# VIS4ROB-lab/HyperSLAM

Hardware: AMD Instinct MI355X
Metric: residual blocks linearised per second (LM iteration = linearise + Schur + solve + update), 128-control-point window (higher is better)
Workload: dtype f64

## Files before the change

hyperslam_amd/csrc/host_structure.hpp:

```cpp
#pragma once
#include <algorithm>
#include <cmath>
#include <cstdint>
#include <numeric>
#include <string>
#include <vector>

#include "../../include/hyperslam_hip.h"
#include "device_math.hpp"

namespace hs {

inline double h_binom(int n, int r) {
  if (r < 0 || r > n) return 0.0;
  double v = 1.0;
  for (int i = 1; i <= r; ++i) v = v * (n - r + i) / i;
  return v;
}

inline hsd::BasisCoef make_basis_coef(int k) {
  hsd::BasisCoef b;
  for (double& v : b.c) v = 0.0;
  std::vector<double> M(size_t(k) * k, 0.0);
  double fact = 1.0;
// ... 189 lines not shown

inline void order_chunks_for_dispatch(const VisualStructure& vs, int k, int n_cu, std::vector<int>* ch_desc, int n) {
  if (n <= 1 || n_cu <= 0) return;
  std::vector<int> weight(n), order(n);
  std::vector<int> cnt;
  for (int c = 0; c < n; ++c) {
    const int* d = ch_desc->data() + 8 * c;
    cnt.assign(size_t(vs.bw) + k + 1, 0);
    for (int q = d[3]; q < d[3] + d[4]; ++q) {
      const int o = vs.first[q] - d[2];
      if (o >= 0 && o < vs.bw) cnt[o]++;
    }
    int run = 0, best = 0;
    for (int o = 0; o < vs.bw + k; ++o) {
      run += (o < vs.bw ? cnt[o] : 0) - (o >= k ? cnt[o - k] : 0);
      best = std::max(best, run);
    }
    weight[c] = best, order[c] = c;
  }
  std::stable_sort(order.begin(), order.end(), [&](int a, int b) { return weight[a] > weight[b]; });
  std::vector<int> slot_chunk(n, -1);
  if (n > n_cu && n <= 2 * n_cu) {
    const int n_lone = 2 * n_cu - n, n_pair = n - n_cu;
    for (int i = 0; i < n_lone; ++i) slot_chunk[n_pair + i] = order[i];
    for (int i = 0; i < n_pair; ++i) slot_chunk[i] = order[n_lone + i], slot_chunk[n_cu + i] = order[n - 1 - i];
  } else {
    for (int i = 0; i < n; ++i) slot_chunk[i] = order[i];
  }
  std::vector<int> out(ch_desc->size(), 0);
  for (int w = 0; w < n; ++w) std::copy(ch_desc->begin() + 8 * slot_chunk[w], ch_desc->begin() + 8 * slot_chunk[w] + 8, out.begin() + 8 * w);
  ch_desc->swap(out);
}

template <class LdsBytes>
inline bool choose_build_geometry(int k, int R0, int L0, size_t lds_two, size_t lds_one, LdsBytes lds_bytes, int* R, int* L) {
  for (const size_t cap : {lds_two, lds_one}) {
    int r = R0, l = L0;
    while (lds_bytes(r, l) > cap && l > 4) --l;
    while (lds_bytes(r, l) > cap && r > 64) r -= 32;
    if (lds_bytes(r, l) <= cap) {
      *R = r, *L = l;
      return true;
    }
  }
  (void)k;
  return false;
}

}
```

hyperslam_amd/csrc/host_tables.hpp:

```cpp
#pragma once
#include <dlfcn.h>
#include <hip/hip_runtime.h>
#include <rccl/rccl.h>

#include <array>
#include <cstdio>
#include <cstdlib>
#include <chrono>
#include <cstring>
#include <string>
#include <mutex>
#include <vector>

#include "host_structure.hpp"
#include "kernels.hpp"

using namespace hs;

namespace {

struct UploadBatch {
  struct Seg {
    unsigned long long dst, off, bytes;
  };
// ... 224 lines not shown
  const void* zeroed_ptr[5] = {nullptr, nullptr, nullptr, nullptr, nullptr};

  VisualStructure vs;
  std::vector<int> pr_order;
  std::vector<int> pr_first, pr_seg_ptr;

  DBuf<double> d_cp, d_cp_cand, d_cam, d_sensor, d_lm, d_lm_cand;
  DBuf<uint8_t> d_cp_const, d_lm_const;
  DBuf<int> d_lm_ptr, d_lm_cfirst, d_lm_ncp, d_lm_yoff, d_cf_ptr;
  DBuf<double> d_lm_scale, d_lm_L, d_lm_yhat, d_lm_sb, d_lm_D2, d_lm_part, d_lm_gmax, d_gabs, d_Y;
  DBuf<double> d_v_stamp, d_v_meas, d_v_rec, d_v_rec_alt;
  DBuf<int> d_v_lm, d_v_info, d_v_first, d_v_pos, d_v_seg_ptr, d_v_dbgpos;
  DBuf<double> d_p_stamp, d_p_meas, d_p_rec;
  DBuf<double> d_i_stamp, d_i_meas, d_i_rec, d_bias_g, d_bias_a, d_bias_g_cand, d_bias_a_cand, d_gravity, d_gravity_cand;
  DBuf<int> d_i_first, d_i_first_bias, d_i_seg_ptr;
  DBuf<ImuParams> d_imu;
  std::vector<int> in_order, in_first, in_first_bias, in_seg_ptr, in_bias_ptr;
  int nb_ine = 0;
  DBuf<int> d_p_sensor, d_p_first, d_p_seg_ptr;
  DBuf<double> d_scale_p, d_Sb, d_Ub, d_Ubk, d_g_s, d_g_full, d_D2p, d_step_p, d_delta_p;
  DBuf<double> d_cost_part, d_cand_part, d_norm_part, d_dbg, d_dbg_cost;
  DBuf<DevState> d_state;
  DBuf<double> d_xbuf, d_xpart, d_segP, d_grpQ, d_Qw, d_Yt, d_gravity_part;
  int yt_stride = 0;
  bool wide_q = false;
  DBuf<double> d_Vb, d_Vb2, d_yt, d_yt2;
  DBuf<double> d_Mb, d_Mb2;
  DBuf<double> d_Sb2, d_g2, d_Ub2, d_Ubk2, d_ybuf2, d_win, d_xsol;
  DBuf<unsigned> d_join;
  DBuf<double> d_dense_ut;
  DBuf<double> d_bf_handover;
  unsigned join_epoch = 0;
  DBuf<int> d_gw_ptr, d_gw_cf, d_sw_ptr, d_sw_seg;
  int n_seg_wg = 0, n_group_wg = 0;
  bool fused = false;
  int dense_border_nb = -1;
  bool bookkeep = false;
  int build_R = 0, build_L = 0;
  size_t build_lds = 0;
  DBuf<int> d_ch_ptr, d_ch_desc;
  DBuf<double> d_ch_gmax;
  std::vector<int> h_ch_ptr, h_gw_ptr, h_gw_cf, h_ch_desc;
  DBuf<double> d_ybuf, d_scale_b, d_Spb, d_Sbb, d_gb_s, d_D2b, d_Zb, d_Cb, d_hb, d_xb, d_delta_b, d_bias_g_snap, d_bias_a_snap, d_gravity_snap;
  DBuf<int> d_i_bias_ptr, d_bfwd_start;
  int n_split = 1;
  int rank = 0, world = 1, min_bw = 0;
  DBuf<double> d_cp_snap, d_lm_snap;
  bool has_snapshot = false;
  DevState* h_state = nullptr;
  bool cov_valid = false;
  int cov_np = 0, cov_ncb = 0, cov_nb = 0, cov_nlm = 0;
  DBuf<double> d_cov_U, d_cov_sig, d_cov_Z, d_cov_X, d_cov_C, d_cov_Li, d_cov_band, d_cov_pb, d_cov_bb, d_cov_lm;
  DBuf<uint8_t> d_cov_const;
  DBuf<int> d_cov_status, d_cov_lm_status;
  int nc = 0;
  std::vector<int> calib_map;
  DBuf<int> d_calib_map;
  DBuf<double> d_calib_rec, d_calib_Yc, d_calib_part, d_cam_cand;
  DBuf<int> d_calib_bfwd;
  int ni = 0;
  std::vector<int> imucal_map;
  DBuf<int> d_imucal_map;
  DBuf<double> d_imucal_rec, d_imucal_part;
  bool imu_estimation = false;
  bool imu_covariance = false;
  bool imu_estimated() const { return ni > 0 && imu_estimation; }
// ... 530 lines not shown
    const int n_seg_ = p->n_cp - k + 1, nca = 6 * k, ntile = vs.bw * (vs.bw + 1) / 2;
    std::vector<int> sw_ptr(n_seg_ + 1, 0), sw_seg;
    for (int f = 0; f < n_seg_; ++f) {
      const int load = (p->fused ? 0 : vs.seg_ptr[f + 1] - vs.seg_ptr[f]) + 3 * (p->pr_seg_ptr[f + 1] - p->pr_seg_ptr[f]) +
                       (p->in_seg_ptr.empty() ? 0 : 3 * (p->in_seg_ptr[f + 1] - p->in_seg_ptr[f]));
      const int nw = p->fused ? (load + 95) / 96 : std::max(1, (load + 95) / 96);
      sw_ptr[f + 1] = sw_ptr[f] + nw;
      for (int w = 0; w < nw; ++w) sw_seg.push_back(f);
    }
    p->n_seg_wg = sw_ptr[n_seg_];
    sw_seg.push_back(0);
    HIP_TRY(p->d_sw_ptr.upload(sw_ptr, s));
    HIP_TRY(p->d_sw_seg.upload(sw_seg, s));
    const int per_wg = 12;
    std::vector<int> gw_ptr(p->n_cp + 1, 0), gw_cf;
    if (!(what & hs_problem::kVis)) {
    } else if (p->fused) {
      HIP_TRY(p->d_gw_ptr.upload(p->h_gw_ptr, s));
      HIP_TRY(p->d_gw_cf.upload(p->h_gw_cf, s));
      HIP_TRY(p->d_ch_ptr.upload(p->h_ch_ptr, s));
      HIP_TRY(p->d_ch_desc.upload(p->h_ch_desc, s));
      p->n_group_wg = int(p->h_ch_ptr.size()) - 1;
    } else {
      for (int c = 0; c < p->n_cp; ++c) {
        const int cnt = vs.cf_ptr[c + 1] - vs.cf_ptr[c], nw = (cnt + per_wg - 1) / per_wg;
        gw_ptr[c + 1] = gw_ptr[c] + nw;
        for (int w = 0; w < nw; ++w) gw_cf.push_back(c);
      }
      p->n_group_wg = gw_ptr[p->n_cp];
      gw_cf.push_back(0);
      HIP_TRY(p->d_gw_ptr.upload(gw_ptr, s));
      HIP_TRY(p->d_gw_cf.upload(gw_cf, s));
    }
    HIP_TRY(p->d_segP.reserve(size_t(p->n_seg_wg) * (size_t(nca) * nca + nca) + 1));
    HIP_TRY(p->d_grpQ.reserve(size_t(p->n_group_wg) * (size_t(ntile) * 36 + (p->fused ? 3 : 1) * 6 * vs.bw) + 1));
    {
      const char* env = std::getenv("HS_WIDE_Q");
      p->wide_q = p->fused && ntile > kBlock && !(env && std::atoi(env) == 0);
      if (p->wide_q) {
        HIP_TRY(p->d_Qw.reserve(size_t(6) * p->n_cp * (6 * vs.bw + 1) + 1));
        p->yt_stride = (p->n_lm + 63) / 64 * 64;
        HIP_TRY(p->d_Yt.reserve(size_t(18) * p->n_cp * p->yt_stride + 2));
      }
    }
  }
  HIP_TRY(p->d_state.reserve(1));

  Tables& T = p->T;
  std::memset(&T, 0, sizeof(T));
  p->dense_border_nb = -1;
  T.sp = Spline{k, p->n_cp, p->t0, p->dt, 1.0 / p->dt, p->rot_const, p->trans_const};
  T.basis = make_basis_coef(k);
  T.cp = p->d_cp.p, T.cp_cand = p->d_cp_cand.p, T.cp_const = p->d_cp_const.p;
  T.cam = p->d_cam.p, T.n_cam = p->n_cam, T.sensor = p->d_sensor.p;
  T.n_lm = p->n_lm, T.lm = p->d_lm.p, T.lm_cand = p->d_lm_cand.p, T.lm_const = p->d_lm_const.p;
  T.lm_ptr = p->d_lm_ptr.p, T.lm_cfirst = p->d_lm_cfirst.p, T.lm_ncp = p->d_lm_ncp.p, T.lm_yoff = p->d_lm_yoff.p, T.cf_ptr = p->d_cf_ptr.p;
  T.lm_scale = p->d_lm_scale.p, T.lm_L = p->d_lm_L.p, T.lm_yhat = p->d_lm_yhat.p, T.lm_sb = p->d_lm_sb.p, T.lm_D2 = p->d_lm_D2.p;
  T.lm_part = p->d_lm_part.p, T.n_lm_part = p->fused ? p->nb_vis : (p->n_lm + kBlock / 64 - 1) / (kBlock / 64), T.lm_gmax = p->d_lm_gmax.p, T.Y = p->d_Y.p;
  {
    int n_obs = p->n_lm;
    while (n_obs > 0 && vs.lm_ptr[n_obs] == vs.lm_ptr[n_obs - 1]) --n_obs;
    T.n_obs_lm = n_obs;
  }
  T.n_vis = n_vis, T.v_stamp = p->d_v_stamp.p, T.v_meas = p->d_v_meas.p, T.v_lm = p->d_v_lm.p, T.v_info = p->d_v_info.p;
  T.v_first = p->d_v_first.p, T.v_pos = p->d_v_pos.p, T.v_rec = p->d_v_rec.p, T.v_rec_alt = p->d_v_rec_alt.p, T.v_seg_ptr = p->d_v_seg_ptr.p;
  T.n_pri = n_pri, T.p_stamp = p->d_p_stamp.p, T.p_meas = p->d_p_meas.p, T.p_sensor = p->d_p_sensor.p, T.p_first = p->d_p_first.p;
  T.p_rec = p->d_p_rec.p, T.p_seg_ptr = p->d_p_seg_ptr.p;
  T.n_ine = n_ine, T.i_stamp = p->d_i_stamp.p, T.i_meas = p->d_i_meas.p, T.i_first = p->d_i_first.p, T.i_first_bias = p->d_i_first_bias.p;
  T.i_rec = p->d_i_rec.p, T.i_seg_ptr = p->d_i_seg_ptr.p, T.imu = p->d_imu.p;
  T.bias_basis = make_basis_coef(p->kb), T.kb = p->kb, T.n_bias = p->has_imu ? p->n_bias : 0, T.bias_t0 = p->bias_t0, T.bias_dt = p->bias_dt;
  T.bias_g = p->d_bias_g.p, T.bias_a = p->d_bias_a.p, T.bias_g_cand = p->d_bias_g_cand.p, T.bias_a_cand = p->d_bias_a_cand.p;
  T.gravity = p->d_gravity.p, T.gravity_cand = p->d_gravity_cand.p, T.bias_const = p->bias_const, T.gravity_const = p->gravity_const;
  T.inertial_literal = p->inertial_mode == HS_INERTIAL_AS_REFERENCE;
  T.nb = (p->has_imu ? 6 * p->n_bias + 2 : 0) + p->ni + p->nc;
  T.nc = p->nc, T.calib_map = p->d_calib_map.p, T.calib_rec = p->d_calib_rec.p, T.calib_Yc = p->d_calib_Yc.p, T.calib_part = p->d_calib_part.p;
  T.n_seg = n_seg, T.bw = vs.bw, T.np = np;
  T.scale_p = p->d_scale_p.p, T.Sb = p->d_Sb.p, T.Ub = p->d_Ub.p, T.Ubk = p->d_Ubk.p, T.g_s = p->d_g_s.p, T.g_full = p->d_g_full.p, T.D2p = p->d_D2p.p, T.gabs = p->d_gabs.p;
  T.step_p = p->d_step_p.p, T.delta_p = p->d_delta_p.p;
  T.cost_part = p->d_cost_part.p, T.cand_part = p->d_cand_part.p, T.n_cost_part = p->nb_vis + p->nb_pri + p->nb_ine;
  if (size_t(T.n_cost_part) > p->d_cost_part.cap || size_t(T.n_cost_part) > p->d_cand_part.cap)
    HS_FAIL(HS_ERR_DEVICE, "internal: cost partial tables shorter than the grids that write them");
  T.norm_part = p->d_norm_part.p, T.n_norm_part = nb_norm;
  T.xbuf = p->d_xbuf.p;
  T.xpart = p->d_xpart.p, T.gravity_part = p->d_gravity_part.p, T.segP = p->d_segP.p, T.grpQ = p->d_grpQ.p, T.Qw = p->d_Qw.p, T.wide_q = p->wide_q && n_vis > 0 ? 1 : 0, T.Yt = p->d_Yt.p, T.yt_stride = p->yt_stride, T.gw_ptr = p->d_gw_ptr.p, T.gw_cf = p->d_gw_cf.p, T.sw_ptr = p->d_sw_ptr.p, T.sw_seg = p->d_sw_seg.p;
  T.xo_g = np * ncb, T.xo_gs = T.xo_g + np, T.xo_dj = T.xo_gs + np, T.xo_pb = T.xo_dj + np, T.xo_bb = T.xo_pb + np * nbd;
  T.xo_gb = T.xo_bb + nbd * nbd, T.xo_cost = T.xo_gb + nbd, T.xo_gmax = T.xo_cost + 1;
  T.ybuf = p->d_ybuf.p, T.ybuf2 = nullptr, T.y_split = np;
  T.fj[0] = FactorJob{T.Sb, T.g_s, T.Ub, T.Ubk, T.ybuf, nullptr, np / 6, -1};
  T.fj[1] = FactorJob{nullptr, nullptr, nullptr, nullptr, nullptr, nullptr, 0, -1};
  T.xsol = p->d_xsol.p, T.join_flag = p->d_join.p, T.join_epoch = 0;
  {
    const long long flags = std::getenv("HS_DEBUG_FLAGS") ? std::atoll(std::getenv("HS_DEBUG_FLAGS")) : 0;
    T.debug_flags = int(flags), T.debug_flags2 = flags > 0 ? int(flags >> 32) : 0;
  }
  {
    const bool two_ended = la_kernel_fits(vs.bw) && np / 6 >= 4 * vs.bw;
    const bool need = two_ended || (HS_AB(T, sw::factor_mfma) && mfma_window_tiles(vs.bw) > 0);
    T.Sb2 = need ? p->d_Sb2.p : nullptr, T.g2 = need ? p->d_g2.p : nullptr;
  }
  T.scale_b = p->d_scale_b.p, T.Spb = p->d_Spb.p, T.Sbb = p->d_Sbb.p, T.gb_s = p->d_gb_s.p, T.D2b = p->d_D2b.p;
  T.Zb = p->d_Zb.p, T.Cb = p->d_Cb.p, T.hb = p->d_hb.p, T.xb = p->d_xb.p, T.delta_b = p->d_delta_b.p, T.i_bias_ptr = p->d_i_bias_ptr.p, T.bfwd_start = (p->nc || est_i) ? p->d_calib_bfwd.p : p->d_bfwd_start.p;
  T.x_count1 = x_count1, T.xo_dec = x_count1, T.xo_cdj = x_count0;
  T.fused = p->fused ? 1 : 0, T.n_chunk = p->fused ? p->n_group_wg : 0, T.ch_ptr = p->d_ch_ptr.p, T.ch_desc = p->d_ch_desc.p;
  T.build_stream_lg = p->fused ? build_streams_packed(vs.bw, k) : 0;
  T.ch_gmax = p->d_ch_gmax.p;
  T.rank = p->rank, T.world = p->world;
  T.st = p->d_state.p;
  HIP_TRY(p->batch.flush(s));
  p->changed = 0;
  if (p->host_timing) {
    const auto host_t2 = std::chrono::steady_clock::now();
    p->host_prepare[0] = std::chrono::duration<double, std::milli>(host_t1 - host_t0).count();
    p->host_prepare[1] = std::chrono::duration<double, std::milli>(host_t2 - host_t1).count();
    p->host_ms[0] += p->host_prepare[0], p->host_ms[1] += p->host_prepare[1];
  }
  return HS_OK;
}
// ... 4 lines not shown
```

hyperslam_amd/csrc/kernels_build.hpp:

```cpp
#pragma once
#include "kernels_common.hpp"

namespace hs {

template <int K>
constexpr int build_rec_stride() { return compact_record<K>() + 2; }

__host__ __device__ inline int band_tile_count(int bw, int k) { return k * bw - k * (k - 1) / 2; }
HSD int band_tile_index(int rb, int d, int bw) { return d * bw - d * (d - 1) / 2 + rb; }
struct BuildStreams {
  int ns[hsd::kMaxOrder], off[hsd::kMaxOrder + 1];
};
__host__ __device__ inline BuildStreams build_streams(int bw, int k) {
  BuildStreams b;
  for (int d = 0; d < hsd::kMaxOrder; ++d) b.ns[d] = d < k ? 1 : 0;
  int used = band_tile_count(bw, k);
  bool stuck[hsd::kMaxOrder] = {false, false, false, false, false, false, false, false};
  for (;;) {
    int best = -1;
    for (int d = 0; d < k; ++d)
      if (!stuck[d] && (best < 0 || (k - d) * b.ns[best] > (k - best) * b.ns[d])) best = d;
    if (best < 0) break;
    const bool fits = used + (bw - best) * b.ns[best] <= kBlock && 2 * b.ns[best] <= 8 && (best == 0 || 2 * b.ns[best] <= b.ns[best - 1]);
    if (!fits) {
// ... 161 lines not shown
  double* Linv = smem + lay.linv;
  double* cpart = smem + lay.cpart;
  int* lp = reinterpret_cast<int*>(smem + lay.ints);
  int* l_ncp = lp + Lmax + 1;
  int* l_yoff = l_ncp + Lmax;
  int* seg_start = l_yoff + Lmax;
  int* wave_cnt = seg_start + bw + 2;
  int* slot_lm = wave_cnt + 4 * bw;
  int* pos = slot_lm + R;
  uint8_t* frozen = reinterpret_cast<uint8_t*>(pos + nseg * (Lmax + 1));
  int* lane_tile = pos + nseg * (Lmax + 1) + (bw + 3) / 4;

  const bool bprof = prof_enabled(T.debug_flags, sw::stamp_build) && lane == 0 && w < 1023;
  long long* blog = reinterpret_cast<long long*>(T.xpart) + 48 * 1024 + 64 * w + 16 * wave;
#define HS_BSTAMP(i) \
  if (bprof) blog[i] = wall_clock64()
  HS_BSTAMP(0);

  const int lo = d0.x, nl = d0.y, cf = d0.z, q0 = d0.w;
  const int rt = R > 128 ? tid : wave == 0 ? lane : wave == 2 ? 64 + lane : kBlock;
  const bool has_rec = rt < nres;
  int my_o = -1, my_l = 0;
  VisualIn in;
  int camid = 0;
  if (has_rec) {
    const int q = q0 + rt;
    in.first = T.v_first[q], my_l = T.v_lm[q] - lo;
    my_o = in.first - cf;
    const int info = T.v_info[q];
    in.type = info >> 16, camid = info & 0xffff;
    in.stamp = T.v_stamp[q];
    in.meas[0] = T.v_meas[3 * q], in.meas[1] = T.v_meas[3 * q + 1], in.meas[2] = T.v_meas[3 * q + 2];
  }
  double f_c0x = 0.0, f_c0y = 0.0, f_c1x = 0.0, f_c1y = 0.0;
  double f_l0x = 0.0, f_l0y = 0.0, f_l0z = 0.0, f_l1x = 0.0, f_l1y = 0.0, f_l1z = 0.0;
  const int ncp_w = min(bw, T.sp.n_cp - cf);
  if (fold) {
    st_spec = st->spec;
    if (w >= T.n_chunk) {
      if (tid == 0) T.cost_part[w] = 0.0, T.ch_gmax[w] = 0.0;
      return;
    }
    st_ready = 1;
    if (tid < 4 * ncp_w) {
      const double2 c0 = reinterpret_cast<const double2*>(T.cp + 8 * cf)[tid], c1 = reinterpret_cast<const double2*>(T.cp_cand + 8 * cf)[tid];
      f_c0x = c0.x, f_c0y = c0.y, f_c1x = c1.x, f_c1y = c1.y;
    }
    if (tid < nl) {
      const double *l0 = T.lm + 3 * (lo + tid), *l1 = T.lm_cand + 3 * (lo + tid);
      f_l0x = l0[0], f_l0y = l0[1], f_l0z = l0[2], f_l1x = l1[0], f_l1y = l1[1], f_l1z = l1[2];
    }
  }
  const bool fresh = !st_ready;
  {
    if (tid < ncp_w) frozen[tid] = T.cp_const[cf + tid];
    for (int e = tid; e < 16 * min(T.n_cam, kBuildCams); e += kBlock) cams[e] = T.cam[e];
    if (tid <= nl) lp[tid] = T.lm_ptr[lo + tid] - q0;
    if (tid < nl) {
      const int dl = lo + tid;
      l_ncp[tid] = T.lm_ncp[dl], l_yoff[tid] = T.lm_yoff[dl];
      double* li = Linv + kLinv * tid;
      li[6] = fresh ? 1.0 : T.lm_scale[3 * dl], li[7] = fresh ? 1.0 : T.lm_scale[3 * dl + 1], li[8] = fresh ? 1.0 : T.lm_scale[3 * dl + 2];
      li[9] = T.lm_const[dl] ? 0.0 : 1.0;
    }
    if (!fold) {
      const bool pend = st_spec == 4 && st_accepted;
      const double* lm_src = pend ? T.lm_cand : T.lm;
      const double2* s2 = reinterpret_cast<const double2*>(T.cp + 8 * cf);
      for (int e = tid; e < 4 * ncp_w; e += kBlock) reinterpret_cast<double2*>(cps_l)[e] = s2[e];
      if (tid < nl) lmp[4 * tid] = lm_src[3 * (lo + tid)], lmp[4 * tid + 1] = lm_src[3 * (lo + tid) + 1], lmp[4 * tid + 2] = lm_src[3 * (lo + tid) + 2];
    }
  }
  int my_rank = 0;
  for (int o = 0; o < nseg; ++o) {
    const unsigned long long m = __ballot(my_o == o);
    if (my_o == o) my_rank = __popcll(m & ((1ull << lane) - 1ull));
    if (lane == 0) wave_cnt[wave * bw + o] = __popcll(m);
  }
  __syncthreads();
  HS_BSTAMP(1);
  if (wave == 1 && !fold) {
    if (lane + 1 < ncp_w) relp[lane] = rel_precompute(cps_l + 8 * lane, cps_l + 8 * lane + 8);
  }
  if (wave == 0) {
    const int tot = lane < nseg ? wave_cnt[lane] + wave_cnt[bw + lane] + wave_cnt[2 * bw + lane] + wave_cnt[3 * bw + lane] : 0;
    int inc = tot;
#pragma unroll
    for (int d = 1; d < 64; d <<= 1) {
      const int up = __shfl_up(inc, d);
      if (lane >= d) inc += up;
    }
    if (lane < nseg) seg_start[lane + 1] = inc;
    if (lane == 0) seg_start[0] = 0;
  }
  __syncthreads();
  int my_slot = 0;
  if (has_rec) {
    my_slot = seg_start[my_o] + my_rank;
    for (int ww = 0; ww < wave; ++ww) my_slot += wave_cnt[ww * bw + my_o];
    slot_lm[my_slot] = my_l;
  }
  for (int e = tid; e < nseg * (Lmax + 1); e += kBlock) pos[e] = seg_start[e / (Lmax + 1) + 1];
  if (fold) {
    const unsigned f = fold_wait(T, reinterpret_cast<unsigned*>(cpart));
    radius = __hip_atomic_load(&st->radius, __ATOMIC_RELAXED, __HIP_MEMORY_SCOPE_AGENT);
    if ((f >> 1) & 1) return;
    const bool acc = f & 1;
    if (tid < 4 * ncp_w) reinterpret_cast<double2*>(cps_l)[tid] = make_double2(acc ? f_c1x : f_c0x, acc ? f_c1y : f_c0y);
    if (tid < nl) lmp[4 * tid] = acc ? f_l1x : f_l0x, lmp[4 * tid + 1] = acc ? f_l1y : f_l0y, lmp[4 * tid + 2] = acc ? f_l1z : f_l0z;
    __syncthreads();
    if (wave == 1 && lane + 1 < ncp_w) relp[lane] = rel_precompute(cps_l + 8 * lane, cps_l + 8 * lane + 8);
  }
  __syncthreads();
  HS_BSTAMP(2);
  const bool dyn = nband <= 64 && !(HS_PROFILE_HOOKS && T.debug_flags < 0);
  if (dyn && wave == 3) {
    int t_rb = lane, t_d = 0;
#pragma unroll
    for (int d = 0; d + 1 < K; ++d)
      if (t_d == d && t_rb >= bw - d) t_rb -= bw - d, t_d = d + 1;
    const bool t_ok = lane < nband;
    int cnt = 0;
    if (t_ok) {
      const int o_hi = min(t_rb, nseg - 1), o_lo = max(0, t_rb + t_d - K + 1);
      if (o_hi >= o_lo) cnt = seg_start[o_hi + 1] - seg_start[o_lo];
    }
    constexpr int kCand[14] = {2, 3, 4, 5, 6, 7, 8, 10, 12, 16, 24, 32, 64, 256};
    int lg_sel = 0;
    bool found = false;
#pragma unroll
    for (int c = 0; c < 14; ++c) {
      const int q = (cnt + kCand[c] - 1) / kCand[c];
      const int lg = (q > 1) + (q > 2) + (q > 4) + (q > 8);
      const int lanes = __popcll(__ballot(t_ok && lg == 0)) + 2 * __popcll(__ballot(t_ok && lg == 1)) + 4 * __popcll(__ballot(t_ok && lg == 2)) +
                        8 * __popcll(__ballot(t_ok && lg == 3)) + 16 * __popcll(__ballot(t_ok && lg == 4));
      if (!found && lanes <= kBlock) found = true, lg_sel = lg;
    }
    int base = 0, my_off = 0;
#pragma unroll
    for (int c = 4; c >= 0; --c) {
      const unsigned long long m = __ballot(t_ok && lg_sel == c);
      if (t_ok && lg_sel == c) my_off = base + (__popcll(m & ((1ull << lane) - 1ull)) << c);
      base += __popcll(m) << c;
    }
#pragma unroll
    for (int j = 0; j < kBlock / 64; ++j) lane_tile[64 * j + lane] = -1;
    wait_lds();
    if (t_ok)
      for (int e = 0; e < (1 << lg_sel); ++e) lane_tile[my_off + e] = t_rb | (t_d << 8) | (lg_sel << 12);
  }
  if (has_rec) {
    const int l_prev = my_slot > seg_start[my_o] ? slot_lm[my_slot - 1] : -1;
    for (int l = l_prev + 1; l <= my_l; ++l) pos[my_o * (Lmax + 1) + l] = my_slot;
    double* rec = recs + my_slot * CS;
    in.cam = camid < kBuildCams ? cams + 16 * camid : T.cam + kCamStride * camid;
    in.lm[0] = lmp[4 * my_l], in.lm[1] = lmp[4 * my_l + 1], in.lm[2] = lmp[4 * my_l + 2];
    const double cost = visual_linearize_compact<K>(T, cps_l - 8 * cf, relp - cf, frozen - cf, in, robustify != 0, rec);
    const double a0 = rec[2], a1 = rec[3], a2 = rec[4], a3 = rec[5], a4 = rec[6], a5 = rec[7], r0 = rec[0], r1 = rec[1];
    double* h = hbr + 10 * rt;
    h[0] = fma(a0, a0, a3 * a3), h[1] = fma(a0, a1, a3 * a4), h[2] = fma(a0, a2, a3 * a5);
    h[3] = fma(a1, a1, a4 * a4), h[4] = fma(a1, a2, a4 * a5), h[5] = fma(a2, a2, a5 * a5);
    h[6] = fma(a0, r0, a3 * r1), h[7] = fma(a1, r0, a4 * r1), h[8] = fma(a2, r0, a5 * r1);
    h[9] = cost;
  }
  HS_BSTAMP(3);
  __syncthreads();
  HS_BSTAMP(4);
  if (tid < 9 * nl) {
    const int l = tid / 9, e = tid - 9 * l;
    double acc = 0.0;
    for (int t = lp[l]; t < lp[l + 1]; ++t) acc += hbr[10 * t + e];
    Hb[10 * l + e] = acc;
  } else if (tid >= kBlock - 8) {
    const int g = tid - (kBlock - 8), per = (nres + 7) / 8;
    double acc = 0.0;
    for (int t = g * per; t < min(nres, (g + 1) * per); ++t) acc += hbr[10 * t + 9];
    cpart[g] = acc;
  }
  __syncthreads();
  const int n_task_w = nl * bw;
  for (int tau = tid; tau < n_task_w; tau += kBlock) {
    const int l = int((unsigned(tau) * bw_magic) >> 20), jb = tau - l * bw;
    double wacc[18];
#pragma unroll
    for (int e = 0; e < 18; ++e) wacc[e] = 0.0;
    int run_lo[K], cum[K];
    int total = 0;
    const bool in_rows = jb < l_ncp[l];
#pragma unroll
    for (int jj = 0; jj < K; ++jj) {
      const int o = jb - jj;
      const bool ok = in_rows && o >= 0 && o < nseg;
      const int* pp = pos + (ok ? o : 0) * (Lmax + 1) + l;
      const int a = pp[0], b = pp[1];
      run_lo[jj] = a, total += ok ? b - a : 0, cum[jj] = total;
    }
#define HS_W_LOAD(h_, dst)                                                   \
// ... 561 lines not shown
```

hyperslam_amd/csrc/kernels_schur.hpp:

```cpp
#pragma once
#include "kernels_common.hpp"

namespace hs {

template <int PS>
HSD void landmark_finish(const Tables& T, int dl, int lane, bool active, bool fresh, double radius, const double* sl_old, int yoff, int rows,
                         const double* h, const double* b, double (*w)[3], bool lead = true) {
  double sl[3];
  if (fresh) {
    sl[0] = 1.0 / (1.0 + sqrt(h[0])), sl[1] = 1.0 / (1.0 + sqrt(h[3])), sl[2] = 1.0 / (1.0 + sqrt(h[5]));
    if (lane < 3 && lead) T.lm_scale[3 * dl + lane] = sl[lane];
  } else {
    sl[0] = sl_old[0], sl[1] = sl_old[1], sl[2] = sl_old[2];
  }
  double v00 = sl[0] * sl[0] * h[0], v01 = sl[0] * sl[1] * h[1], v02 = sl[0] * sl[2] * h[2];
  double v11 = sl[1] * sl[1] * h[3], v12 = sl[1] * sl[2] * h[4], v22 = sl[2] * sl[2] * h[5];
  const double inv_radius = 1.0 / radius;
  const double d0 = fmin(fmax(v00, 1e-6), 1e32) * inv_radius, d1 = fmin(fmax(v11, 1e-6), 1e32) * inv_radius, d2 = fmin(fmax(v22, 1e-6), 1e32) * inv_radius;
  v00 += d0, v11 += d1, v22 += d2;
  auto rsqrt_refined = [](double d) {
    const double y = __builtin_amdgcn_rsq(d);
    const double e = fma(-d * y, y, 1.0);
    return fma(y * e, fma(0.375, e, 0.5), y);
  };
// ... 405 lines not shown
#pragma unroll
    for (int e = 0; e < 36; e += 2) *reinterpret_cast<double2*>(Q + size_t(t) * 36 + e) = make_double2(acc[m][e], acc[m][e + 1]);
    if (t_rb[m] == t_cb[m])
#pragma unroll
      for (int r = 0; r < 6; ++r) Q[size_t(ntile) * 36 + 6 * t_rb[m] + r] = qacc[m][r];
  }
  if (gprof) glog[4] = wall_clock64();
}

template <int NT>
__global__ void __launch_bounds__(kBlock, NT == 1 ? 3 : 1) k_group_gram(Tables T, int batch) {
  group_gram_body<NT>(T, batch, blockIdx.x);
}

template <int K, int NT>
__global__ void __launch_bounds__(kBlock) k_gram_pair(Tables T, int batch, int n_group) {
  if (int(blockIdx.x) < n_group)
    group_gram_body<NT>(T, batch, blockIdx.x);
  else
    seg_gram_body<K>(T, blockIdx.x - n_group);
}

HSD void dense_padding_corner(double* D, int n_dense, int n_pad, int first, int stride);

constexpr int kAsmThreads = 512, kAsmU = 6;

template <int K, int QB, int THREADS>
HSD void assemble_body(const Tables& T, int direct) {
  __shared__ double part[3][THREADS];
  __shared__ double gpair[2];
  const bool aprof = prof_enabled(T.debug_flags, sw::stamp_assemble) && threadIdx.x == 0;
  long long* alog = reinterpret_cast<long long*>(T.xpart) + 128 * 1024 + 8 * (blockIdx.y * gridDim.x + blockIdx.x);
  if (aprof) alog[0] = wall_clock64();
  if (T.st->done) return;
  if (aprof) alog[1] = wall_clock64();
  constexpr int NCA = 6 * K;
  const int i = blockIdx.x, a = blockIdx.y, tid = threadIdx.x;
  const int bw = T.bw, ncb = 6 * bw, R = 6 * bw, ntile = bw * (bw + 1) / 2;
  const size_t pstride = NCA * NCA + NCA, qstride = size_t(ntile) * 36 + (T.fused ? 3 : 1) * R;
  const int f0 = max(0, i - K + 1), f1 = min(i, T.n_seg - 1);
  const int c0 = max(0, i - bw + 1);
  const int nent = ncb + 2;
  const int nent_s = T.wide_q ? 6 * K + 2 : nent;
  const int nsl = max(1, THREADS / nent_s), sl = tid / nent_s, cs = tid % nent_s;
  const int c = T.wide_q ? (cs < 6 * K ? cs : ncb + (cs - 6 * K)) : cs;
  double d_sr = 1.0, d_sc = 1.0, d_radius = 1.0;
  if (direct) {
    d_sr = T.scale_p[6 * i + a];
    if (tid < ncb && 6 * i + tid < T.np) d_sc = T.scale_p[6 * i + tid];
    d_radius = T.st->radius;
  }
  double q_wide = 0.0;
  if (T.wide_q && T.n_lm > 0 && tid < nent && tid != ncb) q_wide = tid < ncb ? (6 * i + tid < T.np ? T.Qw[size_t(6 * i + a) * ncb + tid] : 0.0) : T.Qw[size_t(T.np) * ncb + 6 * i + a];
  double va = 0.0, vb = 0.0;
  double vp = 0.0;
  if (sl < nsl) {
    const int kk = c / 6, cc = c % 6;
    const bool a_live = (c < ncb ? kk < K : c == ncb) && f1 >= f0;
    const bool x_live = T.fused && (c == ncb || c == a);
    const bool b_live = T.n_lm > 0 && (T.wide_q ? (c < ncb && kk < K) || x_live : c < ncb || c == ncb + 1 || x_live);
    const int p_lo = a_live ? T.sw_ptr[f0] : 0, np_ = a_live ? T.sw_ptr[f1 + 1] - p_lo : 0;
    const int q_lo = b_live ? T.gw_ptr[c0] : 0, nq = b_live ? T.gw_ptr[i + 1] - q_lo : 0;
#define HS_SEG_VALUE(p, seg) \
  ((p) < np_ && (c == ncb || i - (seg) + kk < K) \
       ? T.segP[(p_lo + (p)) * int(pstride) + (c == ncb ? NCA * NCA + 6 * (i - (seg)) + a : (6 * (i - (seg)) + a) * NCA + 6 * (i - (seg)) + c)] \
       : 0.0)
#define HS_GRP_VALUE(q, cf) \
  ((q) < nq && (c > ncb || i - (cf) + kk < bw) \
       ? T.grpQ[(q_lo + (q)) * int(qstride) + \
                (c > ncb ? ntile * 36 + 6 * (i - (cf)) + a                                                               \
                 : T.fused ? group_tile_index(i - (cf), i - (cf), bw) * 36 + a * 6 * (bw - (i - (cf))) + c  \
                           : group_tile_index(i - (cf), i - (cf) + kk, bw) * 36 + 6 * a + cc)] \
       : 0.0)
#define HS_GRP_EXTRA(q, cf) ((q) < nq ? T.grpQ[(q_lo + (q)) * int(qstride) + ntile * 36 + (c == ncb ? 1 : 2) * R + 6 * (i - (cf)) + a] : 0.0)
    if (aprof && np_ + nq >= 0) alog[2] = wall_clock64();
    int si[kAsmU], gi[2 * kAsmU];
#pragma unroll
    for (int u = 0; u < kAsmU; ++u) si[u] = sl + u * nsl < np_ ? T.sw_seg[p_lo + sl + u * nsl] : 0;
#pragma unroll
    for (int u = 0; u < 2 * kAsmU; ++u) gi[u] = sl + u * nsl < nq ? T.gw_cf[q_lo + sl + u * nsl] : 0;
    if (aprof && si[0] + gi[0] >= 0) alog[3] = wall_clock64();
    double sv[kAsmU], gv[2 * kAsmU];
#pragma unroll
    for (int u = 0; u < kAsmU; ++u) sv[u] = HS_SEG_VALUE(sl + u * nsl, si[u]);
#pragma unroll
    for (int u = 0; u < 2 * kAsmU; ++u) gv[u] = c == ncb && T.fused ? 0.0 : HS_GRP_VALUE(sl + u * nsl, gi[u]);
    if (x_live) {
      double xv[2 * kAsmU];
#pragma unroll
      for (int u = 0; u < 2 * kAsmU; ++u) xv[u] = HS_GRP_EXTRA(sl + u * nsl, gi[u]);
#pragma unroll
      for (int u = 0; u < 2 * kAsmU; ++u) vp += xv[u];
    }
#pragma unroll
    for (int u = 0; u < kAsmU; ++u) va += sv[u];
#pragma unroll
    for (int u = 0; u < 2 * kAsmU; ++u) vb += gv[u];
    for (int p0 = sl + kAsmU * nsl; p0 < np_; p0 += kAsmU * nsl) {
      double v[kAsmU];
#pragma unroll
      for (int u = 0; u < kAsmU; ++u) {
        const int p = p0 + u * nsl;
        const int seg = p < np_ ? T.sw_seg[p_lo + p] : 0;
        v[u] = HS_SEG_VALUE(p, seg);
      }
#pragma unroll
      for (int u = 0; u < kAsmU; ++u) va += v[u];
    }
    if constexpr (QB == 0) {
      for (int q0 = sl + 2 * kAsmU * nsl; q0 < nq; q0 += kAsmU * nsl) {
        double v[kAsmU];
#pragma unroll
        for (int u = 0; u < kAsmU; ++u) {
          const int q = q0 + u * nsl;
          const int cf = q < nq ? T.gw_cf[q_lo + q] : 0;
          v[u] = c == ncb && T.fused ? 0.0 : HS_GRP_VALUE(q, cf);
          if (x_live) vp += HS_GRP_EXTRA(q, cf);
        }
#pragma unroll
        for (int u = 0; u < kAsmU; ++u) vb += v[u];
      }
    } else {
      int q0 = sl + 2 * kAsmU * nsl;
      int cfn[QB > 0 ? QB : 1];
#pragma unroll
      for (int u = 0; u < QB; ++u) cfn[u] = q0 + u * nsl < nq ? T.gw_cf[q_lo + q0 + u * nsl] : 0;
      for (; q0 < nq; q0 += QB * nsl) {
        double v[QB > 0 ? QB : 1], xv[QB > 0 ? QB : 1];
        int cfc[QB > 0 ? QB : 1];
#pragma unroll
        for (int u = 0; u < QB; ++u) cfc[u] = cfn[u];
#pragma unroll
        for (int u = 0; u < QB; ++u) v[u] = c == ncb && T.fused ? 0.0 : HS_GRP_VALUE(q0 + u * nsl, cfc[u]);
#pragma unroll
        for (int u = 0; u < QB; ++u) xv[u] = x_live ? HS_GRP_EXTRA(q0 + u * nsl, cfc[u]) : 0.0;
#pragma unroll
        for (int u = 0; u < QB; ++u) {
          const int q = q0 + (QB + u) * nsl;
          cfn[u] = q < nq ? T.gw_cf[q_lo + q] : 0;
        }
#pragma unroll
        for (int u = 0; u < QB; ++u) vb += v[u];
#pragma unroll
        for (int u = 0; u < QB; ++u) vp += xv[u];
      }
    }
#undef HS_SEG_VALUE
#undef HS_GRP_VALUE
#undef HS_GRP_EXTRA
  }
  if (aprof && va + vb + vp != 1e300) alog[4] = wall_clock64();
  part[0][tid] = va, part[1][tid] = vb, part[2][tid] = vp;
  __syncthreads();
  if (aprof) alog[5] = wall_clock64();
  if (tid < nent) {
    double sa = 0.0, sb = 0.0, sx = 0.0;
    const int es = !T.wide_q ? tid : tid < 6 * K ? tid : tid >= ncb ? 6 * K + (tid - ncb) : -1;
    for (int q = 0; q < nsl && es >= 0; ++q) sa += part[0][q * nent_s + es], sb += part[1][q * nent_s + es], sx += part[2][q * nent_s + es];
    const int rho = 6 * i + a;
    sb += q_wide;
    if (direct) {
      if (tid < ncb) {
        const int sigma = 6 * i + tid;
        double out = 0.0;
        if (sigma < T.np) {
          out = d_sr * d_sc * (sa + sb);
          if (tid == a) {
            const double d = sa + sx;
            if (d > 0.0) {
              const double d2 = fmin(fmax(d_sr * d_sr * d, 1e-6), 1e32) / d_radius;
              out += d2;
              T.D2p[rho] = d2;
// ... 271 lines not shown
```

hyperslam_amd/csrc/problem.hpp:

```cpp
#pragma once
#include <hip/hip_runtime.h>
#include <stdint.h>

#include "../../include/hyperslam_hip.h"
#include "device_math.hpp"

namespace hs {

constexpr int kMaxIterations = 64;
constexpr int kCamStride = 16;

struct Spline {
  int k, n_cp;
  double t0, dt, inv_dt;
  int rot_const, trans_const;
};

struct DevState {
  double radius, decrease_factor;
  double cost;
  double cand_cost;
  double local_cost;
  double local_cand;
  double model_cost_change;
// ... 138 lines not shown
  int y_split;
  double* scale_b;
  double* Spb;
  double* Sbb;
  double* gb_s;
  double* D2b;
  double* Zb;
  double* Cb;
  double* hb;
  double* xb;
  double* delta_b;
  const int* i_bias_ptr;
  const int* bfwd_start;
  double* cost_part;
  double* cand_part;
  int n_cost_part;
  double* norm_part;
  int n_norm_part;
  double* xbuf;
  const int* sw_ptr;
  const int* sw_seg;
  FactorJob fj[2];
  MfmaJob mj[2];
  double* Sb2;
  double* g2;
  double* xsol;
  unsigned* join_flag;
  unsigned join_epoch;
  unsigned gather_epoch;
  double* gravity_part;
  double* segP;
  const int* gw_ptr;
  const int* gw_cf;
  double* Qw;
  double* Yt;
  int yt_stride;
  int wide_q;
  double* grpQ;
  double* xpart;
  int xo_g, xo_gs, xo_dj, xo_pb, xo_bb, xo_gb, xo_cost, xo_gmax, xo_dec, x_count1;
  int xo_cdj;
  int fused, n_chunk;
  int build_stream_lg;
  double* ch_gmax;
  int bookkeep;
  int fold_decision;
  unsigned fold_epoch;
  const int* ch_ptr;
  const int* ch_desc;
  double* dense;
  int dense_f0;
  unsigned sweep_epoch;
  int dense_border;
  int rank, world;
  int debug_flags;
  int debug_flags2;
  DevState* st;
};

}
```

Before: 266.5 million.

## Speculatively linearise with candidate state before fold wait; precompute assemble row tables

In the fused build kernel, phase-1 linearisation now runs on the candidate control points and landmarks before waiting for the accept/reject decision. If the step is rejected, it reloads the old state and re-linearises, so accepted steps hide the wait latency and rejected steps pay twice. Separately, the Schur assemble kernel reads a per-row table precomputed on the host (segment and group ranges plus index lists). It also issues those index loads before checking the done flag, which removes dependent pointer-chasing loads from its startup.

Result: faster. 273.4 million, median of 4 (+2.6%).

```diff
diff --git a/hyperslam_amd/csrc/host_structure.hpp b/hyperslam_amd/csrc/host_structure.hpp
--- a/hyperslam_amd/csrc/host_structure.hpp
+++ b/hyperslam_amd/csrc/host_structure.hpp
@@ -245,6 +245,33 @@
   ch_desc->swap(out);
 }
 
+inline void build_assemble_rows(int n_cp, int k, int bw, const std::vector<int>& sw_ptr, const std::vector<int>& sw_seg, const std::vector<int>& gw_ptr,
+                                const std::vector<int>& gw_cf, std::vector<int>* rows, int* n_s, int* n_g) {
+  const int n_seg = n_cp - k + 1;
+  const bool has_g = int(gw_ptr.size()) == n_cp + 1;
+  auto range = [&](int i, int* p_lo, int* np, int* q_lo, int* nq) {
+    const int f0 = std::max(0, i - k + 1), f1 = std::min(i, n_seg - 1), c0 = std::max(0, i - bw + 1);
+    *p_lo = f1 >= f0 ? sw_ptr[f0] : 0, *np = f1 >= f0 ? sw_ptr[f1 + 1] - *p_lo : 0;
+    *q_lo = has_g ? gw_ptr[c0] : 0, *nq = has_g ? gw_ptr[i + 1] - *q_lo : 0;
+  };
+  int ms = 0, mg = 0;
+  for (int i = 0; i < n_cp; ++i) {
+    int p_lo, np, q_lo, nq;
+    range(i, &p_lo, &np, &q_lo, &nq);
+    ms = std::max(ms, np), mg = std::max(mg, nq);
+  }
+  *n_s = ms + 1, *n_g = mg + 1;
+  *n_g += (4 - (*n_s + *n_g) % 4) % 4;
+  const int stride = 4 + *n_s + *n_g;
+  rows->assign(size_t(std::max(n_cp, 1)) * stride, 0);
+  for (int i = 0; i < n_cp; ++i) {
+    int* r = rows->data() + size_t(i) * stride;
+    range(i, &r[0], &r[1], &r[2], &r[3]);
+    for (int p = 0; p < r[1]; ++p) r[4 + p] = sw_seg[r[0] + p];
+    for (int q = 0; q < r[3]; ++q) r[4 + *n_s + q] = gw_cf[r[2] + q];
+  }
+}
+
 template <class LdsBytes>
 inline bool choose_build_geometry(int k, int R0, int L0, size_t lds_two, size_t lds_one, LdsBytes lds_bytes, int* R, int* L) {
   for (const size_t cap : {lds_two, lds_one}) {
diff --git a/hyperslam_amd/csrc/host_tables.hpp b/hyperslam_amd/csrc/host_tables.hpp
--- a/hyperslam_amd/csrc/host_tables.hpp
+++ b/hyperslam_amd/csrc/host_tables.hpp
@@ -280,6 +280,8 @@
   DBuf<double> d_bf_handover;
   unsigned join_epoch = 0;
   DBuf<int> d_gw_ptr, d_gw_cf, d_sw_ptr, d_sw_seg;
+  DBuf<int> d_asm_rows;
+  int asm_ns = 0, asm_ng = 0;
   int n_seg_wg = 0, n_group_wg = 0;
   bool fused = false;
   int dense_border_nb = -1;
@@ -876,6 +878,12 @@
       HIP_TRY(p->d_gw_ptr.upload(gw_ptr, s));
       HIP_TRY(p->d_gw_cf.upload(gw_cf, s));
     }
+    p->asm_ns = p->asm_ng = 0;
+    if (p->fused && p->n_cp > 0) {
+      std::vector<int> rows;
+      build_assemble_rows(p->n_cp, k, vs.bw, sw_ptr, sw_seg, p->h_gw_ptr, p->h_gw_cf, &rows, &p->asm_ns, &p->asm_ng);
+      HIP_TRY(p->d_asm_rows.upload(rows, s));
+    }
     HIP_TRY(p->d_segP.reserve(size_t(p->n_seg_wg) * (size_t(nca) * nca + nca) + 1));
     HIP_TRY(p->d_grpQ.reserve(size_t(p->n_group_wg) * (size_t(ntile) * 36 + (p->fused ? 3 : 1) * 6 * vs.bw) + 1));
     {
@@ -927,6 +935,7 @@
   T.norm_part = p->d_norm_part.p, T.n_norm_part = nb_norm;
   T.xbuf = p->d_xbuf.p;
   T.xpart = p->d_xpart.p, T.gravity_part = p->d_gravity_part.p, T.segP = p->d_segP.p, T.grpQ = p->d_grpQ.p, T.Qw = p->d_Qw.p, T.wide_q = p->wide_q && n_vis > 0 ? 1 : 0, T.Yt = p->d_Yt.p, T.yt_stride = p->yt_stride, T.gw_ptr = p->d_gw_ptr.p, T.gw_cf = p->d_gw_cf.p, T.sw_ptr = p->d_sw_ptr.p, T.sw_seg = p->d_sw_seg.p;
+  T.asm_rows = p->asm_ns > 0 ? p->d_asm_rows.p : nullptr, T.asm_ns = p->asm_ns, T.asm_ng = p->asm_ng;
   T.xo_g = np * ncb, T.xo_gs = T.xo_g + np, T.xo_dj = T.xo_gs + np, T.xo_pb = T.xo_dj + np, T.xo_bb = T.xo_pb + np * nbd;
   T.xo_gb = T.xo_bb + nbd * nbd, T.xo_cost = T.xo_gb + nbd, T.xo_gmax = T.xo_cost + 1;
   T.ybuf = p->d_ybuf.p, T.ybuf2 = nullptr, T.y_split = np;
diff --git a/hyperslam_amd/csrc/kernels_build.hpp b/hyperslam_amd/csrc/kernels_build.hpp
--- a/hyperslam_amd/csrc/kernels_build.hpp
+++ b/hyperslam_amd/csrc/kernels_build.hpp
@@ -217,8 +217,6 @@
     in.stamp = T.v_stamp[q];
     in.meas[0] = T.v_meas[3 * q], in.meas[1] = T.v_meas[3 * q + 1], in.meas[2] = T.v_meas[3 * q + 2];
   }
-  double f_c0x = 0.0, f_c0y = 0.0, f_c1x = 0.0, f_c1y = 0.0;
-  double f_l0x = 0.0, f_l0y = 0.0, f_l0z = 0.0, f_l1x = 0.0, f_l1y = 0.0, f_l1z = 0.0;
   const int ncp_w = min(bw, T.sp.n_cp - cf);
   if (fold) {
     st_spec = st->spec;
@@ -227,14 +225,6 @@
       return;
     }
     st_ready = 1;
-    if (tid < 4 * ncp_w) {
-      const double2 c0 = reinterpret_cast<const double2*>(T.cp + 8 * cf)[tid], c1 = reinterpret_cast<const double2*>(T.cp_cand + 8 * cf)[tid];
-      f_c0x = c0.x, f_c0y = c0.y, f_c1x = c1.x, f_c1y = c1.y;
-    }
-    if (tid < nl) {
-      const double *l0 = T.lm + 3 * (lo + tid), *l1 = T.lm_cand + 3 * (lo + tid);
-      f_l0x = l0[0], f_l0y = l0[1], f_l0z = l0[2], f_l1x = l1[0], f_l1y = l1[1], f_l1z = l1[2];
-    }
   }
   const bool fresh = !st_ready;
   {
@@ -248,10 +238,10 @@
       li[6] = fresh ? 1.0 : T.lm_scale[3 * dl], li[7] = fresh ? 1.0 : T.lm_scale[3 * dl + 1], li[8] = fresh ? 1.0 : T.lm_scale[3 * dl + 2];
       li[9] = T.lm_const[dl] ? 0.0 : 1.0;
     }
-    if (!fold) {
+    {
       const bool pend = st_spec == 4 && st_accepted;
-      const double* lm_src = pend ? T.lm_cand : T.lm;
-      const double2* s2 = reinterpret_cast<const double2*>(T.cp + 8 * cf);
+      const double* lm_src = fold || pend ? T.lm_cand : T.lm;
+      const double2* s2 = reinterpret_cast<const double2*>((fold ? T.cp_cand : T.cp) + 8 * cf);
       for (int e = tid; e < 4 * ncp_w; e += kBlock) reinterpret_cast<double2*>(cps_l)[e] = s2[e];
       if (tid < nl) lmp[4 * tid] = lm_src[3 * (lo + tid)], lmp[4 * tid + 1] = lm_src[3 * (lo + tid) + 1], lmp[4 * tid + 2] = lm_src[3 * (lo + tid) + 2];
     }
@@ -264,7 +254,7 @@
   }
   __syncthreads();
   HS_BSTAMP(1);
-  if (wave == 1 && !fold) {
+  if (wave == 1) {
     if (lane + 1 < ncp_w) relp[lane] = rel_precompute(cps_l + 8 * lane, cps_l + 8 * lane + 8);
   }
   if (wave == 0) {
@@ -286,16 +276,6 @@
     slot_lm[my_slot] = my_l;
   }
   for (int e = tid; e < nseg * (Lmax + 1); e += kBlock) pos[e] = seg_start[e / (Lmax + 1) + 1];
-  if (fold) {
-    const unsigned f = fold_wait(T, reinterpret_cast<unsigned*>(cpart));
-    radius = __hip_atomic_load(&st->radius, __ATOMIC_RELAXED, __HIP_MEMORY_SCOPE_AGENT);
-    if ((f >> 1) & 1) return;
-    const bool acc = f & 1;
-    if (tid < 4 * ncp_w) reinterpret_cast<double2*>(cps_l)[tid] = make_double2(acc ? f_c1x : f_c0x, acc ? f_c1y : f_c0y);
-    if (tid < nl) lmp[4 * tid] = acc ? f_l1x : f_l0x, lmp[4 * tid + 1] = acc ? f_l1y : f_l0y, lmp[4 * tid + 2] = acc ? f_l1z : f_l0z;
-    __syncthreads();
-    if (wave == 1 && lane + 1 < ncp_w) relp[lane] = rel_precompute(cps_l + 8 * lane, cps_l + 8 * lane + 8);
-  }
   __syncthreads();
   HS_BSTAMP(2);
   const bool dyn = nband <= 64 && !(HS_PROFILE_HOOKS && T.debug_flags < 0);
@@ -337,17 +317,46 @@
   if (has_rec) {
     const int l_prev = my_slot > seg_start[my_o] ? slot_lm[my_slot - 1] : -1;
     for (int l = l_prev + 1; l <= my_l; ++l) pos[my_o * (Lmax + 1) + l] = my_slot;
-    double* rec = recs + my_slot * CS;
     in.cam = camid < kBuildCams ? cams + 16 * camid : T.cam + kCamStride * camid;
-    in.lm[0] = lmp[4 * my_l], in.lm[1] = lmp[4 * my_l + 1], in.lm[2] = lmp[4 * my_l + 2];
-    const double cost = visual_linearize_compact<K>(T, cps_l - 8 * cf, relp - cf, frozen - cf, in, robustify != 0, rec);
-    const double a0 = rec[2], a1 = rec[3], a2 = rec[4], a3 = rec[5], a4 = rec[6], a5 = rec[7], r0 = rec[0], r1 = rec[1];
-    double* h = hbr + 10 * rt;
-    h[0] = fma(a0, a0, a3 * a3), h[1] = fma(a0, a1, a3 * a4), h[2] = fma(a0, a2, a3 * a5);
-    h[3] = fma(a1, a1, a4 * a4), h[4] = fma(a1, a2, a4 * a5), h[5] = fma(a2, a2, a5 * a5);
-    h[6] = fma(a0, r0, a3 * r1), h[7] = fma(a1, r0, a4 * r1), h[8] = fma(a2, r0, a5 * r1);
-    h[9] = cost;
-  }
+  }
+#define HS_PHASE1_RECORD()                                                                                                   \
+  if (has_rec) {                                                                                                             \
+    double* rec = recs + my_slot * CS;                                                                                       \
+    in.lm[0] = lmp[4 * my_l], in.lm[1] = lmp[4 * my_l + 1], in.lm[2] = lmp[4 * my_l + 2];                                    \
+                                                                 \
+    const double cost = visual_linearize_compact<K>(T, cps_l - 8 * cf, relp - cf, frozen - cf, in, robustify != 0, rec);     \
+                       \
+    const double a0 = rec[2], a1 = rec[3], a2 = rec[4], a3 = rec[5], a4 = rec[6], a5 = rec[7], r0 = rec[0], r1 = rec[1];     \
+    double* h = hbr + 10 * rt;                                                                                               \
+    h[0] = fma(a0, a0, a3 * a3), h[1] = fma(a0, a1, a3 * a4), h[2] = fma(a0, a2, a3 * a5);                                   \
+    h[3] = fma(a1, a1, a4 * a4), h[4] = fma(a1, a2, a4 * a5), h[5] = fma(a2, a2, a5 * a5);                                   \
+    h[6] = fma(a0, r0, a3 * r1), h[7] = fma(a1, r0, a4 * r1), h[8] = fma(a2, r0, a5 * r1);                                   \
+    h[9] = cost;                                                                                                             \
+  }
+  HS_PHASE1_RECORD();
+  if (fold) {
+    const unsigned f = fold_wait(T, reinterpret_cast<unsigned*>(cpart));
+    radius = __hip_atomic_load(&st->radius, __ATOMIC_RELAXED, __HIP_MEMORY_SCOPE_AGENT);
+    if ((f >> 1) & 1) return;
+    if (!(f & 1)) {
+      if (tid < 4 * ncp_w) reinterpret_cast<double2*>(cps_l)[tid] = reinterpret_cast<const double2*>(T.cp + 8 * cf)[tid];
+      if (tid < nl) lmp[4 * tid] = T.lm[3 * (lo + tid)], lmp[4 * tid + 1] = T.lm[3 * (lo + tid) + 1], lmp[4 * tid + 2] = T.lm[3 * (lo + tid) + 2];
+      if (has_rec) {
+        const int q = q0 + rt;
+        in.first = T.v_first[q], my_l = T.v_lm[q] - lo;
+        const int info = T.v_info[q];
+        in.type = info >> 16, camid = info & 0xffff;
+        in.stamp = T.v_stamp[q];
+        in.meas[0] = T.v_meas[3 * q], in.meas[1] = T.v_meas[3 * q + 1], in.meas[2] = T.v_meas[3 * q + 2];
+        in.cam = camid < kBuildCams ? cams + 16 * camid : T.cam + kCamStride * camid;
+      }
+      __syncthreads();
+      if (wave == 1 && lane + 1 < ncp_w) relp[lane] = rel_precompute(cps_l + 8 * lane, cps_l + 8 * lane + 8);
+      __syncthreads();
+      HS_PHASE1_RECORD();
+    }
+  }
+#undef HS_PHASE1_RECORD
   HS_BSTAMP(3);
   __syncthreads();
   HS_BSTAMP(4);
diff --git a/hyperslam_amd/csrc/kernels_schur.hpp b/hyperslam_amd/csrc/kernels_schur.hpp
--- a/hyperslam_amd/csrc/kernels_schur.hpp
+++ b/hyperslam_amd/csrc/kernels_schur.hpp
@@ -461,8 +461,6 @@
   const bool aprof = prof_enabled(T.debug_flags, sw::stamp_assemble) && threadIdx.x == 0;
   long long* alog = reinterpret_cast<long long*>(T.xpart) + 128 * 1024 + 8 * (blockIdx.y * gridDim.x + blockIdx.x);
   if (aprof) alog[0] = wall_clock64();
-  if (T.st->done) return;
-  if (aprof) alog[1] = wall_clock64();
   constexpr int NCA = 6 * K;
   const int i = blockIdx.x, a = blockIdx.y, tid = threadIdx.x;
   const int bw = T.bw, ncb = 6 * bw, R = 6 * bw, ntile = bw * (bw + 1) / 2;
@@ -473,12 +471,32 @@
   const int nent_s = T.wide_q ? 6 * K + 2 : nent;
   const int nsl = max(1, THREADS / nent_s), sl = tid / nent_s, cs = tid % nent_s;
   const int c = T.wide_q ? (cs < 6 * K ? cs : ncb + (cs - 6 * K)) : cs;
+  int h_plo, h_np, h_qlo, h_nq, n_s1, n_g1;
+  const int *seg_list, *grp_list;
+  if (T.asm_rows) {
+    const int* rowt = T.asm_rows + size_t(i) * (4 + T.asm_ns + T.asm_ng);
+    const int4 h = *reinterpret_cast<const int4*>(rowt);
+    h_plo = h.x, h_np = h.y, h_qlo = h.z, h_nq = h.w;
+    seg_list = rowt + 4, grp_list = rowt + 4 + T.asm_ns, n_s1 = T.asm_ns - 1, n_g1 = T.asm_ng - 1;
+  } else {
+    h_plo = f1 >= f0 ? T.sw_ptr[f0] : 0, h_np = f1 >= f0 ? T.sw_ptr[f1 + 1] - h_plo : 0;
+    h_qlo = T.n_lm > 0 ? T.gw_ptr[c0] : 0, h_nq = T.n_lm > 0 ? T.gw_ptr[i + 1] - h_qlo : 0;
+    seg_list = T.sw_seg + h_plo, grp_list = T.n_lm > 0 ? T.gw_cf + h_qlo : T.sw_seg, n_s1 = h_np, n_g1 = T.n_lm > 0 ? h_nq : 0;
+  }
+  int si[kAsmU], gi[2 * kAsmU];
+#pragma unroll
+  for (int u = 0; u < kAsmU; ++u) si[u] = seg_list[min(sl + u * nsl, n_s1)];
+#pragma unroll
+  for (int u = 0; u < 2 * kAsmU; ++u) gi[u] = grp_list[min(sl + u * nsl, n_g1)];
+  const int st_done = T.st->done;
   double d_sr = 1.0, d_sc = 1.0, d_radius = 1.0;
   if (direct) {
     d_sr = T.scale_p[6 * i + a];
     if (tid < ncb && 6 * i + tid < T.np) d_sc = T.scale_p[6 * i + tid];
     d_radius = T.st->radius;
   }
+  if (st_done) return;
+  if (aprof) alog[1] = wall_clock64();
   double q_wide = 0.0;
   if (T.wide_q && T.n_lm > 0 && tid < nent && tid != ncb) q_wide = tid < ncb ? (6 * i + tid < T.np ? T.Qw[size_t(6 * i + a) * ncb + tid] : 0.0) : T.Qw[size_t(T.np) * ncb + 6 * i + a];
   double va = 0.0, vb = 0.0;
@@ -488,8 +506,7 @@
     const bool a_live = (c < ncb ? kk < K : c == ncb) && f1 >= f0;
     const bool x_live = T.fused && (c == ncb || c == a);
     const bool b_live = T.n_lm > 0 && (T.wide_q ? (c < ncb && kk < K) || x_live : c < ncb || c == ncb + 1 || x_live);
-    const int p_lo = a_live ? T.sw_ptr[f0] : 0, np_ = a_live ? T.sw_ptr[f1 + 1] - p_lo : 0;
-    const int q_lo = b_live ? T.gw_ptr[c0] : 0, nq = b_live ? T.gw_ptr[i + 1] - q_lo : 0;
+    const int p_lo = a_live ? h_plo : 0, np_ = a_live ? h_np : 0, q_lo = b_live ? h_qlo : 0, nq = b_live ? h_nq : 0;
 #define HS_SEG_VALUE(p, seg) \
   ((p) < np_ && (c == ncb || i - (seg) + kk < K) \
        ? T.segP[(p_lo + (p)) * int(pstride) + (c == ncb ? NCA * NCA + 6 * (i - (seg)) + a : (6 * (i - (seg)) + a) * NCA + 6 * (i - (seg)) + c)] \
@@ -503,11 +520,6 @@
        : 0.0)
 #define HS_GRP_EXTRA(q, cf) ((q) < nq ? T.grpQ[(q_lo + (q)) * int(qstride) + ntile * 36 + (c == ncb ? 1 : 2) * R + 6 * (i - (cf)) + a] : 0.0)
     if (aprof && np_ + nq >= 0) alog[2] = wall_clock64();
-    int si[kAsmU], gi[2 * kAsmU];
-#pragma unroll
-    for (int u = 0; u < kAsmU; ++u) si[u] = sl + u * nsl < np_ ? T.sw_seg[p_lo + sl + u * nsl] : 0;
-#pragma unroll
-    for (int u = 0; u < 2 * kAsmU; ++u) gi[u] = sl + u * nsl < nq ? T.gw_cf[q_lo + sl + u * nsl] : 0;
     if (aprof && si[0] + gi[0] >= 0) alog[3] = wall_clock64();
     double sv[kAsmU], gv[2 * kAsmU];
 #pragma unroll
@@ -530,7 +542,7 @@
 #pragma unroll
       for (int u = 0; u < kAsmU; ++u) {
         const int p = p0 + u * nsl;
-        const int seg = p < np_ ? T.sw_seg[p_lo + p] : 0;
+        const int seg = p < np_ ? seg_list[p] : 0;
         v[u] = HS_SEG_VALUE(p, seg);
       }
 #pragma unroll
@@ -542,7 +554,7 @@
 #pragma unroll
         for (int u = 0; u < kAsmU; ++u) {
           const int q = q0 + u * nsl;
-          const int cf = q < nq ? T.gw_cf[q_lo + q] : 0;
+          const int cf = q < nq ? grp_list[q] : 0;
           v[u] = c == ncb && T.fused ? 0.0 : HS_GRP_VALUE(q, cf);
           if (x_live) vp += HS_GRP_EXTRA(q, cf);
         }
@@ -553,7 +565,7 @@
       int q0 = sl + 2 * kAsmU * nsl;
       int cfn[QB > 0 ? QB : 1];
 #pragma unroll
-      for (int u = 0; u < QB; ++u) cfn[u] = q0 + u * nsl < nq ? T.gw_cf[q_lo + q0 + u * nsl] : 0;
+      for (int u = 0; u < QB; ++u) cfn[u] = q0 + u * nsl < nq ? grp_list[q0 + u * nsl] : 0;
       for (; q0 < nq; q0 += QB * nsl) {
         double v[QB > 0 ? QB : 1], xv[QB > 0 ? QB : 1];
         int cfc[QB > 0 ? QB : 1];
@@ -566,7 +578,7 @@
 #pragma unroll
         for (int u = 0; u < QB; ++u) {
           const int q = q0 + (QB + u) * nsl;
-          cfn[u] = q < nq ? T.gw_cf[q_lo + q] : 0;
+          cfn[u] = q < nq ? grp_list[q] : 0;
         }
 #pragma unroll
         for (int u = 0; u < QB; ++u) vb += v[u];
diff --git a/hyperslam_amd/csrc/problem.hpp b/hyperslam_amd/csrc/problem.hpp
--- a/hyperslam_amd/csrc/problem.hpp
+++ b/hyperslam_amd/csrc/problem.hpp
@@ -194,6 +194,8 @@
   double* segP;
   const int* gw_ptr;
   const int* gw_cf;
+  const int* asm_rows;
+  int asm_ns, asm_ng;
   double* Qw;
   double* Yt;
   int yt_stride;
```
